# saptadeb/botLab

Measured on AMD Instinct MI355X. Metric: SLAM steps/sec (map+MCL+A*), higher is better.
Workload: dtype int8 grid / f32 poses with f64 intermediates / int64 weights; 1 GPU; full SLAM step on 200x200 @5cm grid (continuing from the shipped, already built obstacle_slam_10mx10m_5cm map), 100000 particles, 290 rays, A* replan on; particles=100000, rays=290, pipeline_depth=14, planner_lanes=2, planner_batch=6, parallelism=single GPU, collective=none

## Files before the change

### botlab_amd/_capi.py

```python
import ctypes as C
import os

_HERE = os.path.dirname(os.path.abspath(__file__))
LIB_PATH = os.environ.get("BOTLAB_HIP_LIB") or os.path.join(_HERE, "libbotlab_hip.so")


class Pose(C.Structure):
    _fields_ = [("utime", C.c_int64), ("x", C.c_float), ("y", C.c_float), ("theta", C.c_float)]

    def __repr__(self):
        return f"Pose(utime={self.utime}, x={self.x!r}, y={self.y!r}, theta={self.theta!r})"


class Particle(C.Structure):
    _fields_ = [("pose", Pose), ("parent_pose", Pose), ("weight", C.c_double)]


class Lidar(C.Structure):
    _fields_ = [("utime", C.c_int64), ("num_ranges", C.c_int32), ("ranges", C.POINTER(C.c_float)),
                ("thetas", C.POINTER(C.c_float)), ("times", C.POINTER(C.c_int64)),
                ("intensities", C.POINTER(C.c_float))]


class SearchParams(C.Structure):
# ... 227 lines not shown
    "bl_pf_set_exchange_buffers": (C.c_int, [_vp, _vp, _vp]),
    "bl_pf_exchange_rec_ptr": (_vp, [_vp]),
    "bl_pf_init_at_pose": (C.c_int, [_vp, _P(Pose), C.c_uint64]),
    "bl_pf_init_uniform": (C.c_int, [_vp, _vp, _vp, C.c_float, C.c_int64, C.c_uint64]),
    "bl_pf_spread": (C.c_int, [_vp, _P(PfSpread)]),
    "bl_pf_set_recovery": (C.c_int, [_vp, _vp, _vp, _P(PfRecoveryParams)]),
    "bl_pf_recovery_state": (C.c_int, [_vp, _P(PfRecoveryState)]),
    "bl_pf_set_adaptive": (C.c_int, [_vp, _P(PfAdaptiveParams)]),
    "bl_pf_adaptive_state": (C.c_int, [_vp, _P(PfAdaptiveState)]),
    "bl_pf_clusters": (C.c_int, [_vp, _P(PfClusterParams), _P(PfClusters), _vp]),
    "bl_pf_cluster_pose": (C.c_int, [_P(PfCluster), C.c_uint64, _P(PfClusterParams), _P(PfClusterPose)]),
    "bl_pf_set_particles": (C.c_int, [_vp, _vp, _vp]),
    "bl_pf_get_particles": (C.c_int, [_vp, _vp]),
    "bl_pf_set_noise_seed": (C.c_int, [_vp, C.c_uint64]),
    "bl_pf_update": (C.c_int, [_vp, _P(Pose), _P(Lidar), _vp, C.c_int, _vp, _P(Pose)]),
    "bl_pf_update_begin": (C.c_int, [_vp, _P(Pose), _P(Lidar), _vp, C.c_int, _vp, _P(C.c_int)]),
    "bl_pf_update_end": (C.c_int, [_vp, _P(Pose)]),
    "bl_pf_update_action_only": (C.c_int, [_vp, _P(Pose), _vp, _P(Pose)]),
    "bl_pf_pose_estimate": (C.c_int, [_vp, _P(Pose)]),
    "bl_pf_pose_device_ptr": (_vp, [_vp]),
    "bl_pf_estimate_posterior_pose": (C.c_int, [_vp, _vp]),
    "bl_pf_debug_estimate_stats": (C.c_int, [_vp, _vp]),
    "bl_pf_debug_set_finish_generation": (C.c_int, [_vp, C.c_uint32]),
    "bl_pf_set_strict_resampling": (C.c_int, [_vp, C.c_int]),
    "bl_pf_debug_resample": (C.c_int, [_vp, C.c_int, _vp]),
    "bl_pf_debug_enable": (C.c_int, [_vp, C.c_int]),
    "bl_pf_debug_last": (C.c_int, [_vp, _vp, _vp]),
    "bl_pf_debug_uniform_runs": (C.c_int, [_vp, _P(C.c_int)]),
    "bl_debug_trig_addition_probe": (C.c_int, [_vp, C.c_uint64, C.c_uint32, _P(C.c_float), _P(C.c_float), _P(C.c_float), _P(C.c_uint64)]),
    "bl_dist_create": (C.c_int, [_vp, _P(_vp)]),
    "bl_dist_destroy": (None, [_vp]),
    "bl_dist_set_distances": (C.c_int, [_vp, _vp]),
    "bl_dist_download": (C.c_int, [_vp, _vp]),
    "bl_dist_debug_stats": (C.c_int, [_vp, _vp]),
    "bl_dist_forget": (C.c_int, [_vp]),
    "bl_dist_debug_bound": (C.c_int, [_vp, _vp, _vp]),
    "bl_dist_debug_fused": (C.c_int, [_vp, _vp]),
    "bl_dist_shape": (C.c_int, [_vp, _P(C.c_int), _P(C.c_int)]),
    "bl_dist_frame": (C.c_int, [_vp, _P(C.c_float), _P(C.c_float), _P(C.c_float), _P(C.c_float)]),
    "bl_dist_device_ptr": (_vp, [_vp]),
    "bl_dist_create_euclidean": (C.c_int, [_vp, C.c_int, _P(_vp)]),
    "bl_dist_metric": (C.c_int, [_vp, _P(C.c_int), _P(C.c_int)]),
    "bl_dist_download_codes": (C.c_int, [_vp, _vp]),
    "bl_dist_table": (C.c_int, [_vp, _vp, _P(C.c_int)]),
    "bl_astar_search": (C.c_int, [_vp, _vp, _P(Pose), _P(Pose), _P(SearchParams), _vp, C.c_int, _P(C.c_int),
                                  _P(C.c_int64)]),
# ... 174 lines not shown
```

### botlab_amd/csrc/bl_mcl.hip

```cpp
#include <math.h>
#include <stdio.h>
#include <stdlib.h>
#include <string.h>
#include <new>

#include <hip/hip_ext.h>
#define BL_PF_HELPER
#include "bl_internal.h"
#include "bl_mcl_finish.h"

#define MCL_LDS_RAYS 384
#define MCL_BLOCK 512
#define MCL_MIN_BLOCKS 512
#define MCL_ROUND_SHORT_DIV 128
#define MCL_WIN_SMALL_BYTES (64 * 1024)
#define MCL_WIN_MAX 208
#define MCL_WIN_MARGIN 24
#define SCAN_THREADS 256
#define SCAN_ITEMS 2
#define SCAN_TILE (SCAN_THREADS * SCAN_ITEMS)


struct mcl_switches {
    bool no_fused_finish, no_framed, no_mirror_reuse, no_stage_dma, no_stage_x4, no_window, no_fast_trig;
    int window;
};
static mcl_switches mcl_switches_read()
{
    auto set = [](const char* name) { return getenv(name) != nullptr; };
    mcl_switches w;
    w.no_fused_finish = set("BOTLAB_MCL_NO_FUSED_FINISH");
    w.no_framed = set("BOTLAB_MCL_NO_FRAMED");
    w.no_mirror_reuse = set("BOTLAB_MCL_NO_MIRROR_REUSE");
    w.no_stage_dma = set("BOTLAB_MCL_NO_STAGE_DMA");
    w.no_stage_x4 = set("BOTLAB_MCL_NO_STAGE_X4");
    w.no_window = set("BOTLAB_MCL_NO_WINDOW");
    w.no_fast_trig = set("BOTLAB_MCL_NO_FAST_TRIG");
    const char* win = getenv("BOTLAB_MCL_WINDOW");
    w.window = win ? atoi(win) : 0;
    return w;
}

struct bl_pf {
    bl_ctx* ctx;
    int N, lo, hi, n_local;
    float4* rec[2];
    bool rec_external;
    int cur;
    double* tile_partials;
    ss_rec* fin_recs;
    ss_wild* fin_wild;
    int fin_subs_cap;
    mclf_tab_elem* fin_tabs;
    unsigned long long* fin_sync;
    unsigned int fin_gen;
    int fin_last_nrec;
    unsigned long long* prefix;
    float4* parent;
    pf_state* state;
    double* partials;
    int partials_cap;
    int last_blocks, last_tile;
    int last_main_blocks, last_main_particles, last_tail_tile;
    bool fused_finish;
    mcl_switches sw;
    int cus;
    bool debug;
    bool strict;
    void* strict_recs; double* strict_starts;
    bool uniform_now;
    bool updated_now;
    bool prefix_is_strict;
    double w_floor;
    unsigned long long* block_sums;
    int scan_blocks;
    int32_t* dbg_idx;
    int32_t* dbg_like;
    float* d_noise;
    bl_particle_t* d_export;
    int64_t pose_utime, parent_utime;
    bl_pose_xyt_t prev_odom;
    bool action_initialized, moved;
    double rot1, trans, rot2, rot1Std, transStd, rot2Std;
    uint64_t noise_seed;
    uint32_t step;
    bool initialized;
// ... 310 lines not shown
    bl_frame frame;
    const float* ranges;
    const float* thetas;
    const int64_t* times;
    int64_t t_begin; double t_den;
    int R;
    int N, lo, n_local;
    double r;
    double M_inv;
    double rot1, trans, rot2, rot1Std, transStd, rot2Std;
    const float* noise;
    uint32_t seed_lo, seed_hi, step;
    int interp;
    int resample;
    int strict;
    int win_w, win_h;
    int split_log2;
    int pk_ok;
    int theta_simple;
    int fast_trig;
    int stage_dma;
    float max_range_cells;
    int main_blocks, main_particles;
    const struct mcl_shard_tab* sh;
    struct pf_recovery_dev* rc;
};
struct mcl_shard_tab { int world, block; const float4* src[BL_MAX_SHARDS]; const unsigned long long* prefix[BL_MAX_SHARDS]; };

struct pf_recovery_dev {
    double w_slow, w_fast, w_avg, p;
    uint32_t updates, primed;
    unsigned long long t;
    unsigned long long total_at_fold;
    unsigned long long injected_total;
    const uint32_t* list;
    uint32_t F, W, k0, k1;
    double ox, oy, mpc;
};
#define RC_CTR 0x72637679u

__device__ __forceinline__ float4 gl_pose(const uint32_t a[4], uint32_t b0, const uint32_t* list, uint32_t F, uint32_t W,
                                          double ox, double oy, double mpc)
{
    const uint32_t r = (uint32_t)__umul64hi(((unsigned long long)a[0] << 32) | a[1], (unsigned long long)F);
    const uint32_t cell = list[r];
    const uint32_t cx = cell % W, cy = cell / W;
// ... 183 lines not shown
#else
#define MCL_STAMP_HW() do { } while (0)
#endif
extern "C" int bl_debug_mcl_stamps(unsigned long long* out, int n)
{
    return hipMemcpyFromSymbol(out, HIP_SYMBOL(g_mcl_stamps), (size_t)n * MCL_STAMP_SLOTS * 8) == hipSuccess ? 0 : 1;
}
#else
#define MCL_STAMP(k) do { } while (0)
#define MCL_STAMP_T(k, T) do { } while (0)
#define MCL_STAMP_HW() do { } while (0)
#endif

template <int INTERP, int MAP_MODE, bool REC = false>
__global__ __launch_bounds__(MCL_BLOCK) void k_mcl_main(mcl_args a)
{
    extern __shared__ __align__(16) signed char s_dyn[];
    __shared__ double s_part[MCL_BLOCK / 64][5];
    __shared__ map_window s_win;
    __shared__ float4 s_ray[MCL_LDS_RAYS];
    __shared__ float4 s_pp[MCL_BLOCK / 4];
    __shared__ float2 s_pcs[MCL_BLOCK / 4];
    __shared__ int s_acc[MCL_BLOCK / 4];
    const lds_i8_t* s_map = (const lds_i8_t*)s_dyn;
    int* s_map32 = (int*)s_dyn;
    map_window win = {0, 0, 0, 0, 0};
    const int tid = (int)threadIdx.x, lane = tid & 63;
    const int wave = __builtin_amdgcn_readfirstlane(tid >> 6);
    if (MAP_MODE == 1) __builtin_amdgcn_s_setprio(3);
    MCL_STAMP(0);

    if (a.sh && __hip_atomic_load(&a.state->shard_broken, __ATOMIC_RELAXED, __HIP_MEMORY_SCOPE_AGENT)) return;
    const bool tail = (int)blockIdx.x >= a.main_blocks;
    const int sl2 = tail ? 6 : a.split_log2;
    const int split = 1 << sl2;
    const int P = MCL_BLOCK >> sl2;
    const int jbase = tail ? a.main_particles + ((int)blockIdx.x - a.main_blocks) * (MCL_BLOCK >> 6) : (int)blockIdx.x * P;
    const int jl = tid >> sl2;
    const int j = jbase + jl;
    const int sub = tid & (split - 1);
    const bool active = j < a.n_local && (tail || j < a.main_particles);
    const bool shared_pro = !INTERP && sl2 >= 2;
    const int pw = shared_pro ? (P + 63) >> 6 : 0;
    const int n_sw = MCL_BLOCK / 64 - pw;
    const int jp = shared_pro ? jbase + tid : j;
    const bool pro_active = shared_pro ? (tid < P && jp < a.n_local && (tail || jp < a.main_particles)) : active;
    const int mp = a.lo + jp;

    if (MAP_MODE == 2) {
        if (tid == 0) {
            map_window w;
            const bl_pose_xyt_t p = a.state->pose;
            const float ex = (float)((double)p.x + a.trans * cos((double)p.theta + a.rot1));
            const float ey = (float)((double)p.y + a.trans * sin((double)p.theta + a.rot1));
            float gx, gy;
            bl_global_to_grid(ex, ey, a.frame, &gx, &gy);
            const int cx = (gx > -1.0e6f && gx < 1.0e6f) ? (int)gx : 0, cy = (gy > -1.0e6f && gy < 1.0e6f) ? (int)gy : 0;
            w.x0 = max(-4, min(cx - a.win_w / 2, a.framed_stride - 4 - a.win_w)) & ~3;
            w.y0 = max(-MCL_FRAME, min(cy - a.win_h / 2, a.frame.height + MCL_FRAME - a.win_h));
            w.w = a.win_w; w.h = a.win_h; w.stride = a.win_w;
            s_win = w;
        }
        __syncthreads();
        win = s_win;
    }
    if (MAP_MODE == 1) {
        win.stride = ((a.frame.width + 3) & ~3) + 8;
        s_map += MCL_FRAME * win.stride + 4;
    }

    if (wave >= pw) {
        const int sw = wave - pw;
        const int st = tid - pw * 64, n_st = n_sw * 64;
        const int cnt0 = a.R < MCL_LDS_RAYS ? a.R : MCL_LDS_RAYS;
        for (int n = st; n < cnt0; n += n_st) s_ray[n] = ray_table_entry(a.ranges[n], a.thetas[n]);
        MCL_STAMP_T(8, pw * 64);
        if (MAP_MODE == 1) {
            const int wq = win.stride >> 2;
            const int rows = a.frame.height + 2 * MCL_FRAME;
            if (a.framed && a.stage_dma) {
                const int pieces = (wq * rows) >> 2;
                const char* src = (const char*)(a.framed - MCL_FRAME * a.framed_stride - 4);
                for (int p0 = sw * 64; p0 < pieces; p0 += n_sw * 64)
                    if (p0 + lane < pieces)
                        __builtin_amdgcn_global_load_lds((const __attribute__((address_space(1))) void*)(src + (size_t)(p0 + lane) * 16),
                                                         (__attribute__((address_space(3))) void*)((char*)s_map32 + (size_t)p0 * 16), 16, 0, 0);
            } else if ((a.frame.width & 3) == 0 && (a.frame.width >> 2) <= 64 && a.stage_dma) {
                const int wdw = a.frame.width >> 2;
                const int H = a.frame.height;
                for (int ry = sw; ry < rows; ry += n_sw) {
                    const int y = ry - MCL_FRAME;
                    int* row = s_map32 + ry * wq;
                    if (y < 0 || y >= H) {
// ... 26 lines not shown
                    s_map32[i] = v;
                }
            }
        }
        if (MAP_MODE == 2) {
            const int wq = win.w >> 2, fq = a.framed_stride >> 2;
            const int* f32 = (const int*)(a.framed - MCL_FRAME * a.framed_stride - 4);
            const int* org = f32 + (size_t)(win.y0 + MCL_FRAME) * fq + ((win.x0 + 4) >> 2);
            if (wq <= 64 && a.stage_dma) {
                if (lane < wq)
                    for (int ry = sw; ry < win.h; ry += n_sw)
                        __builtin_amdgcn_global_load_lds((const __attribute__((address_space(1))) void*)(org + (size_t)ry * fq + lane),
                                                         (__attribute__((address_space(3))) void*)(s_map32 + ry * wq), 4, 0, 0);
            } else
            stage_rows(s_map32, win.h, wq, 0, wq, sw, n_sw, lane, [&](int ry) -> const int* { return org + (size_t)ry * fq; });
        }
    }

    MCL_STAMP_T(4, pw * 64);
#ifdef MCL_STAMPS
    if (wave >= pw) { asm volatile("s_waitcnt vmcnt(0)" ::: "memory"); }
    MCL_STAMP_T(9, pw * 64);
#endif
    double t_units = 0, t_x = 0, t_y = 0, t_s = 0, t_c = 0;
    float2 pcs_own = make_float2(0.0f, 0.0f);
    float pth_sin = 0.0f, pth_cos = 1.0f;
    int i = mp;
    bool injected = false;
    float4 s = make_float4(0.f, 0.f, 0.f, 0.f);
    float px = 0.f, py = 0.f, pth = 0.f, sx0 = 0.f, sy0 = 0.f;
    double rs_T = 0.0;
    int rs_lo = 0, rs_hi = a.N - 1;
    const mcl_prefix_view pview = {a.sh, a.prefix};
    const int uni_n = a.resample ? a.state->uni_n : 0;
    if (a.resample && (!shared_pro || wave < pw)) {
        if (pro_active) { rs_T = a.r + mp * a.M_inv; if (!a.strict && uni_n <= 0) rs_T *= a.state->S; }
        if (uni_n > 0) { }
        else if (a.sh) resample_bracket(pview, a.N, rs_T, pro_active, lane, &rs_lo, &rs_hi, a.strict != 0);
        else resample_bracket<MCL_BRACKET_Q>(a.prefix, a.N, rs_T, pro_active, lane, &rs_lo, &rs_hi, a.strict != 0, pro_active ? mp : -1);
    }
    MCL_STAMP(5);
    if (pro_active) {
        if (a.resample && uni_n > 0) i = uni_search(a.state, uni_n, rs_T, a.N);
        else if (a.resample) i = a.sh ? resample_bisect(pview, rs_T, rs_lo, rs_hi, a.strict != 0) : resample_bisect(a.prefix, rs_T, rs_lo, rs_hi, a.strict != 0);
        MCL_STAMP(6);
        if (REC) {
            const pf_recovery_dev& rc = *a.rc;
            uint32_t d[4];
            bl_philox4x32((uint32_t)mp, rc.updates, RC_CTR, 2u, rc.k0, rc.k1, d);
            injected = (unsigned long long)d[0] < rc.t;
            if (injected) {
                uint32_t w0[4], w1[4];
                bl_philox4x32((uint32_t)mp, rc.updates, RC_CTR, 0u, rc.k0, rc.k1, w0);
                bl_philox4x32((uint32_t)mp, rc.updates, RC_CTR, 1u, rc.k0, rc.k1, w1);
                s = gl_pose(w0, w1[0], rc.list, rc.F, rc.W, rc.ox, rc.oy, rc.mpc);
                i = -1;
            }
        }
        if (!injected)
        s = mcl_src_at(a, i);
        float n1, n2, n3;
        if (a.noise) {
            n1 = a.noise[3 * jp]; n2 = a.noise[3 * jp + 1]; n3 = a.noise[3 * jp + 2];
        } else {
            float z[3];
            philox_normals3((uint32_t)mp, a.step, a.seed_lo, a.seed_hi, z);
            n1 = (float)(a.rot1 + a.rot1Std * (double)z[0]);
            n2 = (float)(a.trans + a.transStd * (double)z[1]);
            n3 = (float)(a.rot2 + a.rot2Std * (double)z[2]);
        }
        const float head = s.z + n1;
        double hs, hc;
        sincos((double)head, &hs, &hc);
        px = (float)((double)s.x + (double)n2 * hc);
        py = (float)((double)s.y + (double)n2 * hs);
        pth = bl_wrap_to_pi(s.z + n1 + n3);
        if (a.cells) bl_global_to_grid(px, py, a.frame, &sx0, &sy0);
        bl_sincosf(pth, &pth_sin, &pth_cos);
        if (a.cells && a.fast_trig) pcs_own = make_float2(a.frame.cpm * pth_cos, a.frame.cpm * pth_sin);
    }
    if (REC) {
        const unsigned long long b = __builtin_amdgcn_ballot_w64(injected && (shared_pro || sub == 0));
        if (b != 0 && lane == 0) atomicAdd(&a.rc->injected_total, (unsigned long long)__popcll(b));
    }
    const float k2_own = 1.2159e-7f * (__builtin_fmaxf(__builtin_fabsf(sx0), __builtin_fabsf(sy0)) + 8.0f);
    MCL_STAMP(7);
    if (shared_pro && tid < P) { s_pp[tid] = make_float4(pth, sx0, sy0, k2_own); s_pcs[tid] = pcs_own; }
    __syncthreads();
    MCL_STAMP(1);

    float r_pth = pth, r_sx0 = sx0, r_sy0 = sy0, trig_k2 = k2_own;
    float2 r_pcs = pcs_own;
    if (shared_pro) { const float4 e = s_pp[jl]; r_pth = e.x; r_sx0 = e.y; r_sy0 = e.z; trig_k2 = e.w; r_pcs = s_pcs[jl]; }
    const float2_t pcs_ = {r_pcs.x, r_pcs.y};
    const float trig_k1 = a.frame.cpm * (2.04f * (MCL_TRIG_EPS + 2.3842e-7f) + 3.648e-7f);
    const float trig_kh2 = 0.5f - 1.5f * trig_k2 - 1.2e-7f;
    const bool fast_trig = a.fast_trig != 0;
    const int isx0 = (int)r_sx0, isy0 = (int)r_sy0;

    int acc = 0;
    if (a.cells) {
        const bool theta_simple = a.theta_simple != 0;
        const bool pk_lane = !INTERP && a.pk_ok && isx0 >= -8191 && isx0 <= 8191 && isy0 >= -8191 && isy0 <= 8191;
        const short2_t S = {(short)isx0, (short)isy0};
        const float2_t start = {r_sx0, r_sy0};
        const float pth_r = r_pth;
        for (int base = 0; base < a.R; base += MCL_LDS_RAYS) {
            const int cnt = a.R - base < MCL_LDS_RAYS ? a.R - base : MCL_LDS_RAYS;
            if (base > 0) {
                __syncthreads();
                for (int n = tid; n < cnt; n += MCL_BLOCK) s_ray[n] = ray_table_entry(a.ranges[base + n], a.thetas[base + n]);
                __syncthreads();
// ... 27 lines not shown
            } else {
                const bl_pose3 pb = {s.x, s.y, s.z};
                const bl_pose3 pe = {px, py, pth};
                for (int n = sub; n < cnt; n += split) {
                    const float4 rt = s_ray[n];
                    float theta, sx, sy;
                    int isx, isy;
                    if (INTERP) {
                        bl_pose3 rp = bl_interpolate_pose(pb, pe, bl_interp_ratio(a.times[base + n], a.t_begin, a.t_den));
                        theta = bl_wrap_to_pi(rp.theta - rt.y);
                        bl_global_to_grid(rp.x, rp.y, a.frame, &sx, &sy);
                        isx = (int)sx; isy = (int)sy;
                    } else {
                        theta = bl_wrap_to_pi(pth_r - rt.y);
                        sx = r_sx0; sy = r_sy0; isx = isx0; isy = isy0;
                    }
                    float sn, cs;
                    bl_sincosf(theta, &sn, &cs);
                    acc += score_ray_half_units<MAP_MODE>(a.cells, s_map, win, a.frame, sx, sy, isx, isy, rt.x, cs, sn);
                }
            }
        }
    }
    MCL_STAMP(2);
    if (active)
        for (int off = split >> 1; off > 0; off >>= 1) acc += __shfl_xor(acc, off, 64);
    if (shared_pro) {
        if (active && sub == 0) s_acc[jl] = acc;
        __syncthreads();
        if (pro_active) acc = s_acc[tid];
    }
    if (shared_pro ? pro_active : (active && sub == 0)) {
        const uint32_t units = a.cells ? (acc > 0 ? (uint32_t)acc * 1000u : 2u) : __float_as_uint(s.w);
        a.dst[mp] = make_float4(px, py, pth, __uint_as_float(units));
        a.parent[jp] = make_float4(s.x, s.y, s.z, 0.0f);
        if (a.dbg_idx) { a.dbg_idx[jp] = i; a.dbg_like[jp] = acc; }
        const float sth = pth_sin, cth = pth_cos;
        t_units = (double)units;
        t_x = t_units * (double)px;
        t_y = t_units * (double)py;
        t_s = t_units * (double)sth;
        t_c = t_units * (double)cth;
    }
    const int nred = shared_pro ? pw : MCL_BLOCK / 64;
    if (wave < nred) {
        t_units = wave_sum(t_units); t_x = wave_sum(t_x); t_y = wave_sum(t_y); t_s = wave_sum(t_s); t_c = wave_sum(t_c);
        if (lane == 0) { s_part[wave][0] = t_units; s_part[wave][1] = t_x; s_part[wave][2] = t_y; s_part[wave][3] = t_s; s_part[wave][4] = t_c; }
    }
    __syncthreads();
    if (tid < 5) {
        double v = 0;
        for (int w = 0; w < nred; ++w) v += s_part[w][tid];
        a.partials[(size_t)blockIdx.x * 5 + tid] = v;
    }
    MCL_STAMP(3);
    MCL_STAMP_HW();
}

__global__ __launch_bounds__(SCAN_THREADS) void k_scan_tile_sums(const float4* __restrict__ rec, int N,
                                                                 unsigned long long* __restrict__ tile_sums,
                                                                 double* __restrict__ tile_partials, int tile0 = 0,
                                                                 unsigned long long* clear_word = nullptr)
{
    __shared__ unsigned long long s[SCAN_THREADS / 64];
    __shared__ double s_pose[SCAN_THREADS / 64][4];
    if (clear_word && blockIdx.x == 0 && threadIdx.x == 0) *clear_word = 0ull;
    const int tile = tile0 + (int)blockIdx.x;
    const int base = tile * SCAN_TILE + threadIdx.x * SCAN_ITEMS;
    unsigned long long v = 0;
    double e[4] = {0, 0, 0, 0};
    if (tile_partials) {
        for (int k = 0; k < SCAN_ITEMS; ++k)
            if (base + k < N) {
                const float4 r = rec[base + k];
                const uint32_t u = __float_as_uint(r.w);
                v += u;
                float sth, cth;
                bl_sincosf(r.z, &sth, &cth);
// ... 364 lines not shown
    }
    out[t] = bl_bswap32(v);
}

__global__ void k_pf_set_pose(pf_state* state, bl_pose_xyt_t pose, int only_utime)
{
    if (only_utime) state->pose.utime = pose.utime;
    else state->pose = pose;
}

static int pf_alloc(bl_pf* pf)
{
    size_t N = pf->cap, n = pf->cap_local;
    if (!pf->rec[0]) {
        BL_HIP(hipMalloc((void**)&pf->rec[0], N * sizeof(float4)));
        BL_HIP(hipMalloc((void**)&pf->rec[1], N * sizeof(float4)));
    }
    BL_HIP(hipMalloc((void**)&pf->prefix, N * sizeof(unsigned long long)));
    BL_HIP(hipMalloc((void**)&pf->parent, n * sizeof(float4)));
    BL_HIP(hipMalloc((void**)&pf->state, sizeof(pf_state)));
    int blocks = (int)((n * 64 + MCL_BLOCK - 1) / MCL_BLOCK) + 1;
    BL_HIP(hipMalloc((void**)&pf->partials, (size_t)blocks * 5 * sizeof(double)));
    pf->partials_cap = blocks;
    static bool attr_set = false;
    if (!attr_set) {
        const int big = 384 * 384;
        BL_HIP(hipFuncSetAttribute((const void*)k_mcl_main<0, 2>, hipFuncAttributeMaxDynamicSharedMemorySize, big));
        BL_HIP(hipFuncSetAttribute((const void*)k_mcl_finish, hipFuncAttributeMaxDynamicSharedMemorySize, MCLF_LDS_BYTES));
        attr_set = true;
    }
    pf->scan_blocks = (int)((N + SCAN_TILE - 1) / SCAN_TILE);
    BL_HIP(hipMalloc((void**)&pf->block_sums, (size_t)pf->scan_blocks * sizeof(unsigned long long)));
    BL_HIP(hipMalloc((void**)&pf->tile_partials, (size_t)pf->scan_blocks * 5 * sizeof(double)));
    pf->fin_subs_cap = (int)(N / MCLF_SUB) + 4 * (MCLF_WG / 64);
    BL_HIP(hipMalloc((void**)&pf->fin_recs, (size_t)2 * pf->fin_subs_cap * sizeof(ss_rec)));
    if (!getenv("BOTLAB_MCL_NO_WILD")) BL_HIP(hipMalloc((void**)&pf->fin_wild, (size_t)2 * pf->fin_subs_cap * sizeof(ss_wild)));
    BL_HIP(hipMalloc((void**)&pf->fin_tabs, (size_t)2 * MCLF_TSLOTS * MCLF_SUB * sizeof(mclf_tab_elem)));
    BL_HIP(hipMalloc((void**)&pf->fin_sync, MCLF_SYNC_WORDS * sizeof(unsigned long long)));
    BL_HIP(hipMemsetAsync(pf->fin_sync, 0, MCLF_SYNC_WORDS * sizeof(unsigned long long), pf->ctx->stream));
    BL_HIP(hipMalloc((void**)&pf->dbg_idx, n * sizeof(int32_t)));
    BL_HIP(hipMalloc((void**)&pf->dbg_like, n * sizeof(int32_t)));
    BL_HIP(hipMemsetAsync(pf->dbg_idx, 0, n * sizeof(int32_t), pf->ctx->stream));
    BL_HIP(hipMemsetAsync(pf->dbg_like, 0, n * sizeof(int32_t), pf->ctx->stream));
    BL_HIP(hipMemsetAsync(pf->state, 0, sizeof(pf_state), pf->ctx->stream));
    return BL_OK;
}
// ... 8 lines not shown
    memset((void*)pf, 0, sizeof(*pf));
    pf->ctx = ctx;
    pf->N = num_particles; pf->lo = shard_lo; pf->hi = shard_hi; pf->n_local = shard_hi - shard_lo;
    pf->cap = num_particles; pf->cap_local = pf->n_local; pf->ad_next = num_particles;
    {
        volatile double wsum = 0.0;
        for (int i = 0; i < num_particles; ++i) wsum = wsum + 0.001;
        pf->w_floor = 0.001 / wsum;
    }
    pf->noise_seed = 0x243F6A8885A308D3ull;
    pf->sw = mcl_switches_read();
    { int cus = 0; if (hipDeviceGetAttribute(&cus, hipDeviceAttributeMultiprocessorCount, ctx->device) == hipSuccess) pf->cus = cus; }
    *out = pf;
    return BL_OK;
}

extern "C" void bl_pf_destroy(bl_pf* pf)
{
    if (!pf) return;
    (void)hipStreamSynchronize(pf->ctx->stream);
    if (!pf->rec_external) { if (pf->rec[0]) (void)hipFree(pf->rec[0]); if (pf->rec[1]) (void)hipFree(pf->rec[1]); }
    void* ptrs[] = {pf->fin_wild, pf->tile_partials, pf->fin_recs, pf->fin_tabs, pf->fin_sync, pf->prefix, pf->parent, pf->state, pf->partials, pf->block_sums, pf->dbg_idx, pf->dbg_like,
                    pf->d_noise, pf->d_export, pf->sh_xchg, pf->sh_tab, pf->sh_fin, pf->sh_flags, pf->sh_peers_dev, pf->strict_recs, pf->strict_starts,
                    pf->gl_tiles, pf->gl_list, pf->sp_parts, pf->sp_out, pf->cl_mem, pf->rc_list, pf->rc_dev, pf->ad_table};
    for (void* p : ptrs) if (p) (void)hipFree(p);
    if (pf->ad_hcount) { (void)hipHostFree(pf->ad_hcount); (void)hipEventDestroy(pf->ad_ev); }
    delete pf->ad_wfloor;
    delete pf;
}

extern "C" int bl_pf_set_exchange_buffers(bl_pf* pf, void* d_rec0, void* d_rec1)
{
    BL_CHECK_ARG(pf != nullptr && d_rec0 && d_rec1);
    if (pf->prefix) { bl_set_error("exchange buffers must be set before the filter is initialised"); return BL_ERR_STATE; }
    pf->rec[0] = (float4*)d_rec0; pf->rec[1] = (float4*)d_rec1; pf->rec_external = true;
    return BL_OK;
}

extern "C" void* bl_pf_exchange_rec_ptr(bl_pf* pf) { return pf && pf->prefix ? (void*)pf->rec[pf->pending_end ? pf->cur ^ 1 : pf->cur] : nullptr; }
extern "C" const void* bl_pf_pose_device_ptr(bl_pf* pf) { return pf && pf->state ? (const void*)&pf->state->pose : nullptr; }

static double pf_w_floor(const bl_pf* pf)
{
    return (pf->N == pf->cap || !pf->ad_wfloor) ? pf->w_floor : (*pf->ad_wfloor)[pf->N];
}

static void pf_adaptive_fill(bl_pf* pf)
// ... 463 lines not shown
                a.win_h = side < H + 2 * MCL_FRAME ? side : H + 2 * MCL_FRAME;
                lds_bytes = a.win_w * a.win_h;
                mode = 2;
            }
        }
    }
    const int block = MCL_BLOCK;
    a.split_log2 = 0;
    if (map) {
        while (a.split_log2 < 6 && ((int64_t)n_out << a.split_log2) < (int64_t)MCL_MIN_BLOCKS * block) a.split_log2++;
        while (a.split_log2 < 2 && ((int64_t)n_out << a.split_log2) < (int64_t)1400 * block) a.split_log2++;
    }
    while (a.split_log2 > 0 && (1 << a.split_log2) > R) a.split_log2--;
    const int gpb = block >> a.split_log2;
    int64_t main_blocks = ((int64_t)n_out + gpb - 1) / gpb, tail_blocks = 0;
    int64_t main_particles = n_out;
    const int tail_tile = block >> 6;
    if (map) {
        const int cus = pf->cus > 0 ? pf->cus : 256;
        int per_cu = 32 / (block >> 6);
        const int lds_per_wg = lds_bytes + 9 * 1024;
        if ((160 * 1024) / lds_per_wg < per_cu) per_cu = (160 * 1024) / lds_per_wg;
        if (per_cu < 1) per_cu = 1;
        const int64_t round = (int64_t)cus * per_cu - (int64_t)cus * per_cu / MCL_ROUND_SHORT_DIV;
        const int64_t full = main_blocks / round, excess = main_blocks - full * round;
        if (full >= 1 && excess > 0 && excess * 8 < round * 5 && excess * gpb <= 24576) {
            main_blocks = full * round;
            main_particles = main_blocks * gpb;
            tail_blocks = ((int64_t)n_out - main_particles + tail_tile - 1) / tail_tile;
        }
    }
    a.main_blocks = (int)main_blocks; a.main_particles = (int)main_particles;
    a.sh = pf->sh_world > 1 ? pf->sh_tab + pf->cur : nullptr;
    pf->sh_stage_sums = pf->sh_stage_groups = false;
    int blocks = (int)(main_blocks + tail_blocks);
    if (blocks > pf->partials_cap) { bl_set_error("internal: partials buffer too small"); return BL_ERR_STATE; }
    const bool rec_mode = pf->rc_on && map != nullptr && resample != 0 && pf->sh_world <= 1 && pf->n_local == pf->N;
    a.rc = nullptr;
    if (rec_mode) {
        const bl_pf_recovery_params_t& q = pf->rc_p;
        pf->rc_u += 1;
        hipLaunchKernelGGL(k_pf_recovery_fold, dim3(1), dim3(64), 0, ctx->stream, (const pf_state*)pf->state, pf->rc_dev, pf->sensed ? 1 : 0,
                           pf->rc_u, pf->N, q.alpha_slow, q.alpha_fast, q.ratio, q.max_fraction);
        a.rc = pf->rc_dev;
    }
    hipEvent_t e0, e1;
    int rc = bl_timer_pair(ctx, BL_K_MCL_MAIN, &e0, &e1);
    if (rc) return rc;
#define MCL_LAUNCH_REC(M, REC)                                                                                    \
    do {                                                                                                          \
        if (a.interp) hipExtLaunchKernelGGL((k_mcl_main<1, (M) == 2 ? 0 : (M), REC>), dim3(blocks), dim3(block), lds_bytes, ctx->stream, e0, e1, 0, a); \
        else hipExtLaunchKernelGGL((k_mcl_main<0, M, REC>), dim3(blocks), dim3(block), lds_bytes, ctx->stream, e0, e1, 0, a);          \
    } while (0)
#define MCL_LAUNCH(M) do { if (rec_mode) MCL_LAUNCH_REC(M, true); else MCL_LAUNCH_REC(M, false); } while (0)
    if (mode == 0) MCL_LAUNCH(0);
    else if (mode == 1) MCL_LAUNCH(1);
    else MCL_LAUNCH(2);
#undef MCL_LAUNCH
#undef MCL_LAUNCH_REC
    BL_HIP(hipGetLastError());
    rc = bl_timer_commit(ctx, BL_K_MCL_MAIN, e0, e1);
    if (rc) return rc;
    if (resize && n_out != pf->N) {
        pf->N = pf->n_local = pf->hi = n_out;
        pf->scan_blocks = (n_out + SCAN_TILE - 1) / SCAN_TILE;
    }
    if (resize && pf->ad_on) { rc = pf_adaptive_count(pf); if (rc) return rc; }
    pf->last_blocks = blocks;
    pf->last_tile = gpb;
    pf->last_main_blocks = a.main_blocks; pf->last_main_particles = a.main_particles; pf->last_tail_tile = tail_tile;
    pf->fused_finish = (pf->n_local == pf->N) && pf->last_tile >= 1 && pf->last_tile <= mclf_chunk(MCLF_GT_LARGE) && !pf->sw.no_fused_finish;
    return BL_OK;
}

static int pf_fused_args(bl_pf* pf, int which, int64_t utime, mcl_finish_args* f)
{
    f->partials = pf->partials; f->nblocks = pf->last_blocks;
    f->rec = pf->rec[which]; f->N = pf->N;
    f->tile = pf->last_tile; f->main_blocks = pf->last_main_blocks; f->main_particles = pf->last_main_particles;
    f->tail_tile = pf->last_tail_tile > 0 ? pf->last_tail_tile : 1;
    f->prefix = pf->prefix; f->state = pf->state; f->utime = utime;
    return pf_finish_fill(pf, f);
}

static int pf_finish_fused(bl_pf* pf, int which, int64_t utime)
{
    bl_ctx* ctx = pf->ctx;
    mcl_finish_args f;
    const int groups = pf_fused_args(pf, which, utime, &f);
    if (groups < 0) return pf_scan(pf, which, 1, utime);
    hipEvent_t e0, e1;
    int rc = bl_timer_begin(ctx, BL_K_MCL_SCAN, &e0, &e1);
    if (rc) return rc;
// ... 550 lines not shown
        pf->sh_broken = true;
        bl_set_error("a wait for another rank's part of the shard exchange gave up (%u): this update's groups, finish, map store and every "
                     "later resampling did nothing, the particle set is no valid posterior any more; set the shards up again "
                     "(bl_pf_shard_setup) or re-initialise the filter", h.wait_timeouts);
        return BL_ERR_STATE;
    }
    if (h.wait_timeouts != 0) {
        BL_HIP(hipMemsetAsync(&pf->state->wait_timeouts, 0, sizeof(unsigned int), pf->ctx->stream));
        bl_set_error("a wait inside a finish launch gave up (%u): the estimate is not valid", h.wait_timeouts);
        return BL_ERR_STATE;
    }
    return BL_OK;
}

extern "C" int bl_pf_estimate_posterior_pose(bl_pf* pf, bl_pose_xyt_t* out_pose)
{
    BL_CHECK_ARG(pf != nullptr);
    if (!pf->initialized || pf->pending_end) { bl_set_error("filter not initialised or update pending"); return BL_ERR_STATE; }
    if (pf->sh_world > 1) { bl_set_error("estimatePosteriorPose on demand needs the whole record on this device (composed shard)"); return BL_ERR_STATE; }
    BL_HIP(hipSetDevice(pf->ctx->device));
    int rc = pf_scan(pf, pf->cur, 1, pf->pending_utime);
    if (rc) return rc;
    if (out_pose) return bl_pf_pose_estimate(pf, out_pose);
    return BL_OK;
}

extern "C" int bl_pf_debug_estimate_stats(bl_pf* pf, uint32_t* out4)
{
    BL_CHECK_ARG(pf != nullptr && out4 != nullptr && pf->state != nullptr);
    BL_HIP(hipMemcpyAsync(out4, pf->state->chain_stats, 8 * sizeof(uint32_t), hipMemcpyDeviceToHost, pf->ctx->stream));
    BL_HIP(hipStreamSynchronize(pf->ctx->stream));
    if (getenv("BOTLAB_FINISH_LOOKAHEAD")) {
        unsigned int la[2];
        BL_HIP(hipMemcpy(la, pf->state->lookahead, sizeof(la), hipMemcpyDeviceToHost));
        fprintf(stderr, "map updates ahead of the exact pose: %u, run again: %u\n", la[0], la[1]);
        unsigned int ps[2];
        BL_HIP(hipMemcpy(ps, pf->state->pre_stats, sizeof(ps), hipMemcpyDeviceToHost));
        fprintf(stderr, "pre-chain sub-tiles by map / replayed: x %u / %u, y %u / %u\n", ps[0] >> 16, ps[0] & 0xffffu, ps[1] >> 16, ps[1] & 0xffffu);
    }
    if (getenv("BOTLAB_FINISH_STAMPS")) {
        unsigned long long st[6];
        BL_HIP(hipMemcpy(st, pf->state->stamps, sizeof(st), hipMemcpyDeviceToHost));
        unsigned long long gs[8];
        BL_HIP(hipMemcpy(gs, pf->state->gstamps, sizeof(gs), hipMemcpyDeviceToHost));
        fprintf(stderr, "group timeline (us, from the finisher's entry): entry %+.2f", ((long long)gs[0] - (long long)st[0]) * 0.01);
        for (int k = 1; k < 8; ++k) fprintf(stderr, " | +%.2f", (gs[k] - gs[k - 1]) * 0.01);
// ... 632 lines not shown
```

### botlab_amd/host.py

```python
import ctypes as C
import math

import numpy as np

from . import _capi
from ._capi import Lidar, Particle, Pose, SearchParams, check

_libc = C.CDLL(None)
_libc.rand.restype = C.c_int

PARTICLE_DTYPE = np.dtype([("utime", "<i8"), ("x", "<f4"), ("y", "<f4"), ("theta", "<f4"), ("_pad0", "<f4"),
                           ("p_utime", "<i8"), ("p_x", "<f4"), ("p_y", "<f4"), ("p_theta", "<f4"), ("_pad1", "<f4"),
                           ("weight", "<f8")])
POSE_DTYPE = np.dtype([("utime", "<i8"), ("x", "<f4"), ("y", "<f4"), ("theta", "<f4"), ("_pad", "<f4")])
assert PARTICLE_DTYPE.itemsize == 56 and POSE_DTYPE.itemsize == 24


def make_pose(x=0.0, y=0.0, theta=0.0, utime=0):
    return Pose(int(utime), float(np.float32(x)), float(np.float32(y)), float(np.float32(theta)))


class LidarScan:

    def __init__(self, ranges, thetas, times, utime=0):
# ... 341 lines not shown
        return self.ctx.lib.bl_pf_pose_device_ptr(self.h)

    def estimatePosteriorPose(self):
        out = Pose()
        check(self.ctx.lib.bl_pf_estimate_posterior_pose(self.h, C.byref(out)))
        return out

    def setStrictResampling(self, on=True):
        check(self.ctx.lib.bl_pf_set_strict_resampling(self.h, 1 if on else 0))

    def debugResample(self, rand_value):
        idx = np.empty(self._counts()[1] if self._adaptive_used else self.N, np.int32)
        check(self.ctx.lib.bl_pf_debug_resample(self.h, int(rand_value), idx.ctypes.data))
        return idx

    def debugUniformRuns(self):
        n = C.c_int()
        check(self.ctx.lib.bl_pf_debug_uniform_runs(self.h, C.byref(n)))
        return n.value

    def debugEstimateStats(self):
        out = np.zeros(8, np.uint32)
        check(self.ctx.lib.bl_pf_debug_estimate_stats(self.h, out.ctypes.data))
        return [int(v) for v in out]

    def particles(self):
        out = np.zeros(self._counts()[0], dtype=PARTICLE_DTYPE)
        check(self.ctx.lib.bl_pf_get_particles(self.h, out.ctypes.data))
        return out

    def debugEnable(self, on=True):
        check(self.ctx.lib.bl_pf_debug_enable(self.h, 1 if on else 0))

    def debugLast(self):
        n = self._counts()[0]
        idx = np.empty(n, np.int32)
        like = np.empty(n, np.int32)
        check(self.ctx.lib.bl_pf_debug_last(self.h, idx.ctypes.data, like.ctypes.data))
        return idx, like

    def close(self):
        if self.h:
            self.ctx.lib.bl_pf_destroy(self.h)
            self.h = None


# ... 1010 lines not shown
```

### include/botlab_hip.h

```cpp
#ifndef BOTLAB_HIP_H
#define BOTLAB_HIP_H

#include <math.h>
#include <stddef.h>
#include <stdint.h>

#ifdef __cplusplus
extern "C" {
#endif

#define BL_OK 0
#define BL_ERR_HIP 1
#define BL_ERR_ARG 2
#define BL_ERR_CAPACITY 3
#define BL_ERR_STATE 4

const char* bl_last_error(void);
const char* bl_version(void);

typedef struct bl_pose_xyt_t {
    int64_t utime;
    float x, y, theta;
} bl_pose_xyt_t;

// ... 150 lines not shown
        out->mean_y = ((double)ay + my + 0.5) / xy_scale;
        out->var_x = ((double)rxx / dU - mx * mx) / (xy_scale * xy_scale);
        out->var_y = ((double)ryy / dU - my * my) / (xy_scale * xy_scale);
        out->cov_xy = ((double)rxy / dU - mx * my) / (xy_scale * xy_scale);
        out->theta = atan2(dss, dsc);
        out->theta_resultant = hypot(dss, dsc) / (dU * 1048576.0);
    }
    return 1;
}
int bl_pf_set_particles(bl_pf* pf, const bl_particle_t* particles, const uint32_t* units);
int bl_pf_get_particles(bl_pf* pf, bl_particle_t* out_local);
int bl_pf_set_noise_seed(bl_pf* pf, uint64_t seed);

int bl_pf_update(bl_pf* pf, const bl_pose_xyt_t* odometry, const bl_lidar_t* scan, const bl_grid* map, int rand_value,
                 const float* noise, bl_pose_xyt_t* out_pose);
int bl_pf_update_begin(bl_pf* pf, const bl_pose_xyt_t* odometry, const bl_lidar_t* scan, const bl_grid* map,
                       int rand_value, const float* noise, int* moved);
int bl_pf_update_end(bl_pf* pf, bl_pose_xyt_t* out_pose);
int bl_pf_update_action_only(bl_pf* pf, const bl_pose_xyt_t* odometry, const float* noise, bl_pose_xyt_t* out_pose);
int bl_pf_pose_estimate(bl_pf* pf, bl_pose_xyt_t* out_pose);
const void* bl_pf_pose_device_ptr(bl_pf* pf);
int bl_pf_estimate_posterior_pose(bl_pf* pf, bl_pose_xyt_t* out_pose);
int bl_pf_debug_estimate_stats(bl_pf* pf, uint32_t* out8);
int bl_pf_debug_set_finish_generation(bl_pf* pf, uint32_t generation);
int bl_pf_debug_uniform_runs(bl_pf* pf, int* out_runs);
int bl_pf_set_strict_resampling(bl_pf* pf, int on);
int bl_pf_debug_resample(bl_pf* pf, int rand_value, int32_t* out_idx);
int bl_pf_debug_enable(bl_pf* pf, int on);
int bl_debug_trig_addition_probe(bl_ctx* ctx, uint64_t pairs, uint32_t seed, float* max_sin_err, float* max_cos_err, float* eps_used,
                                 uint64_t* pairs_checked);
int bl_pf_debug_last(bl_pf* pf, int32_t* resample_idx, int32_t* likelihood_half_units);

typedef struct bl_scan_match_params_t {
    int32_t nx, ny;
    int32_t ntheta;
    float   dtheta;
    float   max_range;
    int32_t min_score;
    int32_t keep_volume;
} bl_scan_match_params_t;
typedef struct bl_scan_match_result_t {
    bl_pose_xyt_t pose;
    int32_t di, dj, dk;
    int32_t score;
    int32_t score_centre;
    int32_t ties;
// ... 405 lines not shown
```

Measured before the change: 12350 steps/s.

## Replace MCL tail blocks with an atomic work pool drained by main blocks

Instead of launching separate tail blocks after the main round, the MCL kernel launches only the main-round blocks. Each block, after finishing its own particles, claims tail tiles from a global atomic cursor and runs up to two extra pooled passes over them. Per-tile partial sums are written straight to the tail slots. The aim is to remove the under-filled second wave of tail blocks. The cost is extra atomics, a more complex kernel with a lambda-based multipass structure, and possible register-pressure growth.

```diff
diff --git a/botlab_amd/_capi.py b/botlab_amd/_capi.py
--- a/botlab_amd/_capi.py
+++ b/botlab_amd/_capi.py
@@ -273,6 +273,7 @@
     "bl_pf_estimate_posterior_pose": (C.c_int, [_vp, _vp]),
     "bl_pf_debug_estimate_stats": (C.c_int, [_vp, _vp]),
     "bl_pf_debug_set_finish_generation": (C.c_int, [_vp, C.c_uint32]),
+    "bl_pf_debug_launch_shape": (C.c_int, [_vp, _vp]),
     "bl_pf_set_strict_resampling": (C.c_int, [_vp, C.c_int]),
     "bl_pf_debug_resample": (C.c_int, [_vp, C.c_int, _vp]),
     "bl_pf_debug_enable": (C.c_int, [_vp, C.c_int]),
diff --git a/botlab_amd/csrc/bl_mcl.hip b/botlab_amd/csrc/bl_mcl.hip
--- a/botlab_amd/csrc/bl_mcl.hip
+++ b/botlab_amd/csrc/bl_mcl.hip
@@ -12,6 +12,13 @@
 #define MCL_LDS_RAYS 384
 #define MCL_BLOCK 512
 #define MCL_MIN_BLOCKS 512
+#ifndef MCL_POOL_TAKE_LOG2
+#define MCL_POOL_TAKE_LOG2 2
+#endif
+#define MCL_POOL_MAX_TAKES 2
+#ifndef MCL_POOL_MIN_PCT
+#define MCL_POOL_MIN_PCT 0
+#endif
 #define MCL_ROUND_SHORT_DIV 128
 #define MCL_WIN_SMALL_BYTES (64 * 1024)
 #define MCL_WIN_MAX 208
@@ -24,6 +31,8 @@
 struct mcl_switches {
     bool no_fused_finish, no_framed, no_mirror_reuse, no_stage_dma, no_stage_x4, no_window, no_fast_trig;
     int window;
+    bool no_pool;
+    int round;
 };
 static mcl_switches mcl_switches_read()
 {
@@ -38,6 +47,9 @@
     w.no_fast_trig = set("BOTLAB_MCL_NO_FAST_TRIG");
     const char* win = getenv("BOTLAB_MCL_WINDOW");
     w.window = win ? atoi(win) : 0;
+    w.no_pool = set("BOTLAB_MCL_NO_POOL");
+    const char* round = getenv("BOTLAB_MCL_ROUND");
+    w.round = round ? atoi(round) : 0;
     return w;
 }
 
@@ -62,6 +74,9 @@
     int partials_cap;
     int last_blocks, last_tile;
     int last_main_blocks, last_main_particles, last_tail_tile;
+    int last_launched, last_pool_tiles, last_take_tiles, last_tail_blocks;
+    unsigned long long* pool_cursor;
+    unsigned long long pool_base;
     bool fused_finish;
     mcl_switches sw;
     int cus;
@@ -418,6 +433,9 @@
     int stage_dma;
     float max_range_cells;
     int main_blocks, main_particles;
+    unsigned long long* pool_cursor;
+    unsigned long long pool_base;
+    int pool_tiles, pool_takes, pool_take_log2;
     const struct mcl_shard_tab* sh;
     struct pf_recovery_dev* rc;
 };
@@ -647,6 +665,8 @@
     __shared__ float4 s_pp[MCL_BLOCK / 4];
     __shared__ float2 s_pcs[MCL_BLOCK / 4];
     __shared__ int s_acc[MCL_BLOCK / 4];
+    static_assert(((MCL_BLOCK >> 6) << MCL_POOL_TAKE_LOG2) < MCL_BLOCK / 4, "s_take lies behind a take's scores");
+    int& s_take = s_acc[MCL_BLOCK / 4 - 1];
     const lds_i8_t* s_map = (const lds_i8_t*)s_dyn;
     int* s_map32 = (int*)s_dyn;
     map_window win = {0, 0, 0, 0, 0};
@@ -656,21 +676,16 @@
     MCL_STAMP(0);
 
     if (a.sh && __hip_atomic_load(&a.state->shard_broken, __ATOMIC_RELAXED, __HIP_MEMORY_SCOPE_AGENT)) return;
-    const bool tail = (int)blockIdx.x >= a.main_blocks;
-    const int sl2 = tail ? 6 : a.split_log2;
-    const int split = 1 << sl2;
-    const int P = MCL_BLOCK >> sl2;
-    const int jbase = tail ? a.main_particles + ((int)blockIdx.x - a.main_blocks) * (MCL_BLOCK >> 6) : (int)blockIdx.x * P;
-    const int jl = tid >> sl2;
-    const int j = jbase + jl;
-    const int sub = tid & (split - 1);
-    const bool active = j < a.n_local && (tail || j < a.main_particles);
-    const bool shared_pro = !INTERP && sl2 >= 2;
-    const int pw = shared_pro ? (P + 63) >> 6 : 0;
-    const int n_sw = MCL_BLOCK / 64 - pw;
-    const int jp = shared_pro ? jbase + tid : j;
-    const bool pro_active = shared_pro ? (tid < P && jp < a.n_local && (tail || jp < a.main_particles)) : active;
-    const int mp = a.lo + jp;
+    const bool pool = !INTERP && a.pool_cursor != nullptr;
+    bool pooled = false;
+    bool tail = !pool && (int)blockIdx.x >= a.main_blocks;
+    int sl2 = tail ? 6 : a.split_log2;
+    int jbase = tail ? a.main_particles + ((int)blockIdx.x - a.main_blocks) * (MCL_BLOCK >> 6) : (int)blockIdx.x * (MCL_BLOCK >> sl2);
+    int take_own = -1;
+    unsigned long long drawn = 0;
+    int takes_done = 0; (void)takes_done;
+    const int uni_n = a.resample ? a.state->uni_n : 0;
+    const mcl_prefix_view pview = {a.sh, a.prefix};
 
     if (MAP_MODE == 2) {
         if (tid == 0) {
@@ -694,6 +709,9 @@
         s_map += MCL_FRAME * win.stride + 4;
     }
 
+  {
+    const int pw = (!INTERP && sl2 >= 2) ? ((MCL_BLOCK >> sl2) + 63) >> 6 : 0;
+    const int n_sw = MCL_BLOCK / 64 - pw;
     if (wave >= pw) {
         const int sw = wave - pw;
         const int st = tid - pw * 64, n_st = n_sw * 64;
@@ -766,6 +784,20 @@
     if (wave >= pw) { asm volatile("s_waitcnt vmcnt(0)" ::: "memory"); }
     MCL_STAMP_T(9, pw * 64);
 #endif
+  }
+  auto run_pass = [&](const int pass) __attribute__((always_inline)) -> bool {
+    const int split = 1 << sl2;
+    const int P = MCL_BLOCK >> sl2;
+    const int jl = tid >> sl2;
+    int j = jbase + jl;
+    const int sub = tid & (split - 1);
+    bool active = j < a.n_local && (tail || j < a.main_particles);
+    const bool shared_pro = !INTERP && sl2 >= 2;
+    const int pw = shared_pro ? (P + 63) >> 6 : 0;
+    const int jp = shared_pro ? jbase + tid : j;
+    const bool pro_active = shared_pro ? (tid < P && jp < a.n_local && (tail || jp < a.main_particles)) : active;
+    const int mp = a.lo + jp;
+
     double t_units = 0, t_x = 0, t_y = 0, t_s = 0, t_c = 0;
     float2 pcs_own = make_float2(0.0f, 0.0f);
     float pth_sin = 0.0f, pth_cos = 1.0f;
@@ -775,19 +807,17 @@
     float px = 0.f, py = 0.f, pth = 0.f, sx0 = 0.f, sy0 = 0.f;
     double rs_T = 0.0;
     int rs_lo = 0, rs_hi = a.N - 1;
-    const mcl_prefix_view pview = {a.sh, a.prefix};
-    const int uni_n = a.resample ? a.state->uni_n : 0;
     if (a.resample && (!shared_pro || wave < pw)) {
         if (pro_active) { rs_T = a.r + mp * a.M_inv; if (!a.strict && uni_n <= 0) rs_T *= a.state->S; }
         if (uni_n > 0) { }
         else if (a.sh) resample_bracket(pview, a.N, rs_T, pro_active, lane, &rs_lo, &rs_hi, a.strict != 0);
         else resample_bracket<MCL_BRACKET_Q>(a.prefix, a.N, rs_T, pro_active, lane, &rs_lo, &rs_hi, a.strict != 0, pro_active ? mp : -1);
     }
-    MCL_STAMP(5);
+    if (!pooled) MCL_STAMP(5);
     if (pro_active) {
         if (a.resample && uni_n > 0) i = uni_search(a.state, uni_n, rs_T, a.N);
         else if (a.resample) i = a.sh ? resample_bisect(pview, rs_T, rs_lo, rs_hi, a.strict != 0) : resample_bisect(a.prefix, rs_T, rs_lo, rs_hi, a.strict != 0);
-        MCL_STAMP(6);
+        if (!pooled) MCL_STAMP(6);
         if (REC) {
             const pf_recovery_dev& rc = *a.rc;
             uint32_t d[4];
@@ -828,10 +858,22 @@
         if (b != 0 && lane == 0) atomicAdd(&a.rc->injected_total, (unsigned long long)__popcll(b));
     }
     const float k2_own = 1.2159e-7f * (__builtin_fmaxf(__builtin_fabsf(sx0), __builtin_fabsf(sy0)) + 8.0f);
-    MCL_STAMP(7);
+    if (!pooled) MCL_STAMP(7);
     if (shared_pro && tid < P) { s_pp[tid] = make_float4(pth, sx0, sy0, k2_own); s_pcs[tid] = pcs_own; }
+    if (pooled && tid == 0) s_take = take_own;
     __syncthreads();
-    MCL_STAMP(1);
+    if (!pooled) MCL_STAMP(1);
+    if (pooled) {
+        const int t = __builtin_amdgcn_readfirstlane(s_take);
+        if (t < 0) {
+            if (tid == 0 && pass < MCL_POOL_MAX_TAKES)
+                (void)__hip_atomic_fetch_add(a.pool_cursor, (unsigned long long)(MCL_POOL_MAX_TAKES - pass), __ATOMIC_RELAXED, __HIP_MEMORY_SCOPE_AGENT);
+            return false;
+        }
+        jbase = a.main_particles + t * P;
+        j = jbase + jl;
+        active = j < a.n_local;
+    }
 
     float r_pth = pth, r_sx0 = sx0, r_sy0 = sy0, trig_k2 = k2_own;
     float2 r_pcs = pcs_own;
@@ -905,12 +947,13 @@
             }
         }
     }
-    MCL_STAMP(2);
+    if (!pooled) MCL_STAMP(2);
     if (active)
         for (int off = split >> 1; off > 0; off >>= 1) acc += __shfl_xor(acc, off, 64);
     if (shared_pro) {
         if (active && sub == 0) s_acc[jl] = acc;
         __syncthreads();
+        if (pool && tid == 0 && pass < MCL_POOL_MAX_TAKES) drawn = __hip_atomic_fetch_add(a.pool_cursor, 1ull, __ATOMIC_RELAXED, __HIP_MEMORY_SCOPE_AGENT);
         if (pro_active) acc = s_acc[tid];
     }
     if (shared_pro ? pro_active : (active && sub == 0)) {
@@ -925,18 +968,50 @@
         t_s = t_units * (double)sth;
         t_c = t_units * (double)cth;
     }
-    const int nred = shared_pro ? pw : MCL_BLOCK / 64;
-    if (wave < nred) {
-        t_units = wave_sum(t_units); t_x = wave_sum(t_x); t_y = wave_sum(t_y); t_s = wave_sum(t_s); t_c = wave_sum(t_c);
-        if (lane == 0) { s_part[wave][0] = t_units; s_part[wave][1] = t_x; s_part[wave][2] = t_y; s_part[wave][3] = t_s; s_part[wave][4] = t_c; }
-    }
-    __syncthreads();
-    if (tid < 5) {
-        double v = 0;
-        for (int w = 0; w < nred; ++w) v += s_part[w][tid];
-        a.partials[(size_t)blockIdx.x * 5 + tid] = v;
-    }
-    MCL_STAMP(3);
+    if (!pooled) {
+        const int nred = shared_pro ? pw : MCL_BLOCK / 64;
+        if (wave < nred) {
+            t_units = wave_sum(t_units); t_x = wave_sum(t_x); t_y = wave_sum(t_y); t_s = wave_sum(t_s); t_c = wave_sum(t_c);
+            if (lane == 0) { s_part[wave][0] = t_units; s_part[wave][1] = t_x; s_part[wave][2] = t_y; s_part[wave][3] = t_s; s_part[wave][4] = t_c; }
+        }
+        __syncthreads();
+        if (tid < 5 && (!pool || (int)blockIdx.x < a.main_blocks)) {
+            double v = 0;
+            for (int w = 0; w < nred; ++w) v += s_part[w][tid];
+            a.partials[(size_t)blockIdx.x * 5 + tid] = v;
+        }
+        MCL_STAMP(3);
+    } else if (wave == 0) {
+        static_assert(MCL_BLOCK / 64 == 8, "the tile sums below are wave_sum's last three steps");
+        for (int off = 4; off > 0; off >>= 1) {
+            t_units += __shfl_down(t_units, off, 64); t_x += __shfl_down(t_x, off, 64); t_y += __shfl_down(t_y, off, 64);
+            t_s += __shfl_down(t_s, off, 64); t_c += __shfl_down(t_c, off, 64);
+        }
+        const int tile = take_own * (P >> 3) + (lane >> 3);
+        if (lane < P && (lane & 7) == 0 && tile < a.pool_tiles) {
+            double* o = a.partials + (size_t)(a.main_blocks + tile) * 5;
+            o[0] = 0.0 + t_units; o[1] = 0.0 + t_x; o[2] = 0.0 + t_y; o[3] = 0.0 + t_s; o[4] = 0.0 + t_c;
+        }
+    }
+    if (pooled) takes_done++;
+    if (!pool || pass == MCL_POOL_MAX_TAKES) return false;
+    if (!pooled) MCL_STAMP(10);
+    pooled = true; tail = true;
+    sl2 = 6 - a.pool_take_log2;
+    take_own = -1;
+    if (wave == 0) {
+        const unsigned long long d = drawn - a.pool_base;
+        take_own = __builtin_amdgcn_readfirstlane(d < (unsigned long long)a.pool_takes ? (int)d : -1);
+    }
+    jbase = take_own >= 0 ? a.main_particles + take_own * (MCL_BLOCK >> sl2) : a.n_local;
+    return true;
+  };
+  static_assert(MCL_POOL_MAX_TAKES == 2, "one call per pass");
+  if (run_pass(0) && run_pass(1)) run_pass(2);
+#ifdef MCL_STAMPS
+    if (pool && threadIdx.x == 0 && blockIdx.x < 4096)
+        g_mcl_stamps[blockIdx.x * MCL_STAMP_SLOTS + 11] = wall_clock64() | ((unsigned long long)min(takes_done, 255) << 56);
+#endif
     MCL_STAMP_HW();
 }
 
@@ -1347,6 +1422,9 @@
     int blocks = (int)((n * 64 + MCL_BLOCK - 1) / MCL_BLOCK) + 1;
     BL_HIP(hipMalloc((void**)&pf->partials, (size_t)blocks * 5 * sizeof(double)));
     pf->partials_cap = blocks;
+    BL_HIP(hipMalloc((void**)&pf->pool_cursor, sizeof(unsigned long long)));
+    BL_HIP(hipMemsetAsync(pf->pool_cursor, 0, sizeof(unsigned long long), pf->ctx->stream));
+    pf->pool_base = 0;
     static bool attr_set = false;
     if (!attr_set) {
         const int big = 384 * 384;
@@ -1401,7 +1479,7 @@
     if (!pf->rec_external) { if (pf->rec[0]) (void)hipFree(pf->rec[0]); if (pf->rec[1]) (void)hipFree(pf->rec[1]); }
     void* ptrs[] = {pf->fin_wild, pf->tile_partials, pf->fin_recs, pf->fin_tabs, pf->fin_sync, pf->prefix, pf->parent, pf->state, pf->partials, pf->block_sums, pf->dbg_idx, pf->dbg_like,
                     pf->d_noise, pf->d_export, pf->sh_xchg, pf->sh_tab, pf->sh_fin, pf->sh_flags, pf->sh_peers_dev, pf->strict_recs, pf->strict_starts,
-                    pf->gl_tiles, pf->gl_list, pf->sp_parts, pf->sp_out, pf->cl_mem, pf->rc_list, pf->rc_dev, pf->ad_table};
+                    pf->gl_tiles, pf->gl_list, pf->sp_parts, pf->sp_out, pf->cl_mem, pf->rc_list, pf->rc_dev, pf->ad_table, pf->pool_cursor};
     for (void* p : ptrs) if (p) (void)hipFree(p);
     if (pf->ad_hcount) { (void)hipHostFree(pf->ad_hcount); (void)hipEventDestroy(pf->ad_ev); }
     delete pf->ad_wfloor;
@@ -1911,7 +1989,8 @@
         const int lds_per_wg = lds_bytes + 9 * 1024;
         if ((160 * 1024) / lds_per_wg < per_cu) per_cu = (160 * 1024) / lds_per_wg;
         if (per_cu < 1) per_cu = 1;
-        const int64_t round = (int64_t)cus * per_cu - (int64_t)cus * per_cu / MCL_ROUND_SHORT_DIV;
+        int64_t round = (int64_t)cus * per_cu - (int64_t)cus * per_cu / MCL_ROUND_SHORT_DIV;
+        if (pf->sw.round > 0) round = pf->sw.round;
         const int64_t full = main_blocks / round, excess = main_blocks - full * round;
         if (full >= 1 && excess > 0 && excess * 8 < round * 5 && excess * gpb <= 24576) {
             main_blocks = full * round;
@@ -1919,11 +1998,29 @@
             tail_blocks = ((int64_t)n_out - main_particles + tail_tile - 1) / tail_tile;
         }
     }
+    const int64_t round_blocks = main_blocks;
+    auto pool_fits = [&](int64_t tiles) { return ((tiles + (1 << MCL_POOL_TAKE_LOG2) - 1) >> MCL_POOL_TAKE_LOG2) <= (int64_t)MCL_POOL_MAX_TAKES * round_blocks; };
+    const bool pool_ok = tail_blocks > 0 && !pf->sw.no_pool && !a.interp && a.split_log2 >= 2 && R <= MCL_LDS_RAYS && pf->sh_world <= 1 &&
+                         pool_fits(tail_blocks);
+    if (pool_ok && MCL_POOL_MIN_PCT > 0) {
+        const int64_t mb = (int64_t)n_out * (100 - MCL_POOL_MIN_PCT) / 100 / gpb;
+        const int64_t tb = ((int64_t)n_out - mb * gpb + tail_tile - 1) / tail_tile;
+        if (mb >= 1 && mb < main_blocks && pool_fits(tb)) { main_blocks = mb; main_particles = mb * gpb; tail_blocks = tb; }
+    }
     a.main_blocks = (int)main_blocks; a.main_particles = (int)main_particles;
     a.sh = pf->sh_world > 1 ? pf->sh_tab + pf->cur : nullptr;
     pf->sh_stage_sums = pf->sh_stage_groups = false;
     int blocks = (int)(main_blocks + tail_blocks);
     if (blocks > pf->partials_cap) { bl_set_error("internal: partials buffer too small"); return BL_ERR_STATE; }
+    int launched = blocks;
+    a.pool_cursor = nullptr; a.pool_base = 0; a.pool_tiles = 0; a.pool_takes = 0; a.pool_take_log2 = MCL_POOL_TAKE_LOG2;
+    if (pool_ok) {
+        a.pool_cursor = pf->pool_cursor; a.pool_base = pf->pool_base;
+        a.pool_tiles = (int)tail_blocks;
+        a.pool_takes = (a.pool_tiles + (1 << a.pool_take_log2) - 1) >> a.pool_take_log2;
+        launched = (int)round_blocks;
+        pf->pool_base += (unsigned long long)MCL_POOL_MAX_TAKES * (unsigned long long)launched;
+    }
     const bool rec_mode = pf->rc_on && map != nullptr && resample != 0 && pf->sh_world <= 1 && pf->n_local == pf->N;
     a.rc = nullptr;
     if (rec_mode) {
@@ -1938,8 +2035,8 @@
     if (rc) return rc;
 #define MCL_LAUNCH_REC(M, REC)                                                                                    \
     do {                                                                                                          \
-        if (a.interp) hipExtLaunchKernelGGL((k_mcl_main<1, (M) == 2 ? 0 : (M), REC>), dim3(blocks), dim3(block), lds_bytes, ctx->stream, e0, e1, 0, a); \
-        else hipExtLaunchKernelGGL((k_mcl_main<0, M, REC>), dim3(blocks), dim3(block), lds_bytes, ctx->stream, e0, e1, 0, a);          \
+        if (a.interp) hipExtLaunchKernelGGL((k_mcl_main<1, (M) == 2 ? 0 : (M), REC>), dim3(launched), dim3(block), lds_bytes, ctx->stream, e0, e1, 0, a); \
+        else hipExtLaunchKernelGGL((k_mcl_main<0, M, REC>), dim3(launched), dim3(block), lds_bytes, ctx->stream, e0, e1, 0, a);          \
     } while (0)
 #define MCL_LAUNCH(M) do { if (rec_mode) MCL_LAUNCH_REC(M, true); else MCL_LAUNCH_REC(M, false); } while (0)
     if (mode == 0) MCL_LAUNCH(0);
@@ -1958,6 +2055,8 @@
     pf->last_blocks = blocks;
     pf->last_tile = gpb;
     pf->last_main_blocks = a.main_blocks; pf->last_main_particles = a.main_particles; pf->last_tail_tile = tail_tile;
+    pf->last_launched = launched; pf->last_pool_tiles = a.pool_tiles; pf->last_take_tiles = a.pool_cursor ? 1 << a.pool_take_log2 : 0;
+    pf->last_tail_blocks = a.pool_cursor ? 0 : (int)tail_blocks;
     pf->fused_finish = (pf->n_local == pf->N) && pf->last_tile >= 1 && pf->last_tile <= mclf_chunk(MCLF_GT_LARGE) && !pf->sw.no_fused_finish;
     return BL_OK;
 }
@@ -2554,6 +2653,14 @@
     int rc = pf_scan(pf, pf->cur, 1, pf->pending_utime);
     if (rc) return rc;
     if (out_pose) return bl_pf_pose_estimate(pf, out_pose);
+    return BL_OK;
+}
+
+extern "C" int bl_pf_debug_launch_shape(bl_pf* pf, int32_t* out8)
+{
+    BL_CHECK_ARG(pf != nullptr && out8 != nullptr);
+    out8[0] = pf->last_launched; out8[1] = pf->last_main_blocks; out8[2] = pf->last_main_particles; out8[3] = pf->last_tail_tile;
+    out8[4] = pf->last_pool_tiles; out8[5] = pf->last_take_tiles; out8[6] = pf->last_take_tiles > 0 ? 1 : 0; out8[7] = pf->last_tail_blocks;
     return BL_OK;
 }
 
diff --git a/botlab_amd/host.py b/botlab_amd/host.py
--- a/botlab_amd/host.py
+++ b/botlab_amd/host.py
@@ -387,6 +387,11 @@
     def debugEstimateStats(self):
         out = np.zeros(8, np.uint32)
         check(self.ctx.lib.bl_pf_debug_estimate_stats(self.h, out.ctypes.data))
+        return [int(v) for v in out]
+
+    def debugLaunchShape(self):
+        out = np.zeros(8, np.int32)
+        check(self.ctx.lib.bl_pf_debug_launch_shape(self.h, out.ctypes.data))
         return [int(v) for v in out]
 
     def particles(self):
diff --git a/include/botlab_hip.h b/include/botlab_hip.h
--- a/include/botlab_hip.h
+++ b/include/botlab_hip.h
@@ -196,6 +196,7 @@
 const void* bl_pf_pose_device_ptr(bl_pf* pf);
 int bl_pf_estimate_posterior_pose(bl_pf* pf, bl_pose_xyt_t* out_pose);
 int bl_pf_debug_estimate_stats(bl_pf* pf, uint32_t* out8);
+int bl_pf_debug_launch_shape(bl_pf* pf, int32_t* out8);
 int bl_pf_debug_set_finish_generation(bl_pf* pf, uint32_t generation);
 int bl_pf_debug_uniform_runs(bl_pf* pf, int* out_runs);
 int bl_pf_set_strict_resampling(bl_pf* pf, int on);
```

After: 11430 steps/s. -7.4%, worse.
